# abdelhakim96/Dynamic-Obstacle-Avoidance-MPC

Measured on AMD Instinct MI355X. Metric: MPC solves/sec (N=20, 3 obstacles), higher is better.
Workload: dtype f64; 1 GPU; C2: 1024 identical scenarios per GPU, N=20, Tf=2s, 3 moving obstacles; global_batch=1024, per_gpu_batch=1024, N=20, n_obst=3, parallelism=single GPU

## Files before the change

### dynamic-obstacle-avoidance-mpc_amd/csrc/rti_kernel.hpp

```cpp
#pragma once
#include <hip/hip_runtime.h>
#include <stdint.h>
#include <type_traits>

#ifdef MPC_PHASE_TIMING
#define MPC_T0() long long t_prev_ = clock64()
#define MPC_TICK(k) do { const long long t_now_ = clock64(); tacc_[k] += t_now_ - t_prev_; t_prev_ = t_now_; } while (0)
#else
#define MPC_T0() do {} while (0)
#define MPC_TICK(k) do {} while (0)
#endif

namespace mpc {

struct World {
    double xmin, xmax, ymin, ymax;
    int bug_compat_predict;
};

enum : int {
    kFuseShift = 1,
    kFusePlant = 2,
    kFuseObstacles = 4,
    kFuseResetOnFail = 8,
    kFuseAliasBug = 16,
    kFuseMetrics = 32,
    kFuseInterpGuess = 64,
    kFuseAdvanceRef = 128
};

struct KParams {
    int N, batch;
    int n_obst;
    int soft_h, bx_terminal, iter_max;
    double dt, h2;
    double Hd_stage[7];
    double Hd_term[5];
    double Wg[6];
    double Weg[4];
    double bx_lo[4], bx_hi[4], bu_lo[2], bu_hi[2];
    double r2;
    double slack_a, slack_b, ss;
    double tol, mu0, thr0;
    double polish_ratio;
    float polish_tol;
    float polish_kappa;
    float polish_tol_unsolved;
    double polish_res_g;
    double tl_min;
    double mu_div, mu_cap, mu_settled;
    const double *x0, *P, *goal;
    const double *alpha;
    double *X, *U, *u0, *cost;
    int32_t *status, *iters;
    const int32_t *order;
    int32_t *iters_acc, *status_acc;
    const double *obst;
    double *x0_rw, *obst_rw;
    const double *noise;
    double randomness, vmax, tol_goal, r_hit;
    World world;
    int fused;
    double *ep_min_margin;
    int32_t *ep_flags;
    int32_t *ep_steps;
    double *trace;
    const double *yref;
    int32_t *ref_off;
    int ref_T;
};

__device__ __forceinline__ const double *ref_row(const double *yref, const int32_t *off, int T, int inst, int i)
{
    const int32_t *op = off;
    asm volatile("" : "+v"(op));
    const int o = off ? op[inst] : 0;
    int r = o > T - 1 - i ? T - 1 : o + i;
    r = r < 0 ? 0 : r;
    return yref + ((size_t)inst * T + r) * 6;
}

__device__ __forceinline__ void load_ref(const KParams &p, int inst, int i, bool has_u, double r[6])
{
    const double *row = ref_row(p.yref, p.ref_off, p.ref_T, inst, i);
#pragma unroll
    for (int c = 0; c < 4; c++) r[c] = row[c];
    r[4] = has_u ? row[4] : 0.0; r[5] = has_u ? row[5] : 0.0;
}

__device__ __forceinline__ double ls_cost_ref(const double Wg[6], const double Weg[4], const double xi[5], const double ui[2], const double r[6], bool has_u)
{
    const double ex = xi[0] - r[0], ey = xi[1] - r[1], ev = xi[3] - r[2], eo = xi[4] - r[3];
    if (has_u) {
        const double ea = ui[0] - r[4], eal = ui[1] - r[5];
        return 0.5 * (Wg[0] * ex * ex + Wg[1] * ey * ey + Wg[2] * ev * ev + Wg[3] * eo * eo + Wg[4] * ea * ea + Wg[5] * eal * eal);
    }
    return 0.5 * (Weg[0] * ex * ex + Weg[1] * ey * ey + Weg[2] * ev * ev + Weg[3] * eo * eo);
}

static constexpr double kTLMin = 1e-11;
static constexpr double kFracToBoundary = 0.999995;
static constexpr double kMuDiverged = 1e8;
static constexpr double kMuCapFailed = 1e4;
static constexpr int kMuCapSettled = 20;

__device__ static constexpr double kGLC[4] = {0.069431844202973712388, 0.330009478207571867599,
                                              0.669990521792428132401, 0.930568155797026287612};
__device__ static constexpr double kGLB[4] = {0.173927422568726928687, 0.326072577431273071313,
                                              0.326072577431273071313, 0.173927422568726928687};

template <bool JAC>
__device__ __forceinline__ void dyn_step(const double x[5], const double u[2], double dt, double xn[5], double ae[6], double be[4])
{
    const double psi = x[2], v = x[3], om = x[4], a = u[0], al = u[1];
    double sx = 0, sy = 0, xpsi = 0, xv = 0, xom = 0, xa = 0, xal = 0, ypsi = 0, yv = 0, yom = 0, ya = 0, yal = 0;
#pragma unroll
    for (int j = 0; j < 4; j++) {
        const double tau = kGLC[j] * dt, w = kGLB[j] * dt;
        const double vj = v + a * tau;
        const double pj = psi + om * tau + 0.5 * al * tau * tau;
        double sj, cj;
        sincos(pj, &sj, &cj);
        const double wvc = w * vj * cj, wvs = w * vj * sj;
        sx += wvc; sy += wvs;
        if (JAC) {
            const double ht2 = 0.5 * tau * tau;
            xpsi -= wvs;        ypsi += wvc;
            xv += w * cj;       yv += w * sj;
            xom -= wvs * tau;   yom += wvc * tau;
            xa += w * tau * cj; ya += w * tau * sj;
            xal -= wvs * ht2;   yal += wvc * ht2;
        }
    }
    xn[0] = x[0] + sx; xn[1] = x[1] + sy;
    xn[2] = psi + om * dt + 0.5 * al * dt * dt;
    xn[3] = v + a * dt;
    xn[4] = om + al * dt;
    if (JAC) {
        ae[0] = xpsi; ae[1] = xv; ae[2] = xom; ae[3] = ypsi; ae[4] = yv; ae[5] = yom;
        be[0] = xa; be[1] = xal; be[2] = ya; be[3] = yal;
    }
}

__device__ __forceinline__ void coord_advance(double lo, double hi, double dt, double &x, double &v)
{
#pragma clang fp contract(off)
    const double av = fabs(v);
    const double n = v < 0 ? x - lo : hi - x;
    bool hit = false;
    double t_hit = 0.0;
    if (v != 0 && !(n > av * dt * (1.0 + 0x1p-50))) { t_hit = n / av; hit = t_hit <= dt; }
    if (hit) { const double a = v * t_hit, b = v * (dt - t_hit); x = x + (a - b); v = -v; }
    else { const double a = v * dt; x = x + a; }
}
__device__ __forceinline__ void obstacle_advance(const World w, double dt, double &x, double &vx, double &y, double &vy)
{
    coord_advance(w.xmin, w.xmax, dt, x, vx);
    coord_advance(w.ymin, w.ymax, dt, y, vy);
}
__device__ __forceinline__ void interp_guess(const double x0[5], double goal_y, int i, int N, double xg[5])
{
#pragma clang fp contract(off)
    const double dy = goal_y - x0[1];
// ... 2865 lines not shown
```

### dynamic-obstacle-avoidance-mpc_amd/csrc/rti_split_kernel.hpp

```cpp
#pragma once
#include "rti_kernel.hpp"
#include <type_traits>

namespace mpc {

template <int LPS, int NOBST, bool W2 = false, bool BLK2 = false>
struct SplitLds {
    using LT = typename std::conditional<W2, RowLdsC, RowLds>::type;
    static constexpr int NBL = 6 / LPS;
    static constexpr int NSL = (NOBST + LPS - 1) / LPS;
    static __host__ __device__ constexpr int results(int N) { return W2 ? 0 : (N + 1) * RowLds::HS; }
    static __host__ __device__ constexpr int total(int N, bool lookahead)
    {
        if (BLK2) return Blk2Lds::total(N) + (lookahead ? (N + 1) * NOBST * 2 : 0);
        return LT::total(N, 1) + results(N) + ((lookahead && !W2) ? (N + 1) * NOBST * 2 : 0);
    }
};

template <int K>
__device__ __forceinline__ double nth_of_six(double a0, double a1, double a2, double a3, double a4, double a5)
{
    if constexpr (K == 0) return a0; else if constexpr (K == 1) return a1; else if constexpr (K == 2) return a2;
    else if constexpr (K == 3) return a3; else if constexpr (K == 4) return a4; else return a5;
}

#ifdef MPC_FORCE_WAVES2
#define MPC_SPLIT_BOUNDS(W2) __launch_bounds__(64, 2)
#else
#define MPC_SPLIT_BOUNDS(W2) __launch_bounds__(64, (W2) ? 2 : 1)
#endif
template <int NOBST, int LPS, bool W2 = false, bool MASKED = false, bool BLK2 = false, bool REF = false>
__global__ MPC_SPLIT_BOUNDS(W2) void rti_split_kernel(const KParams p)
{
    static_assert(!REF || !BLK2, "the per-stage reference is not built for the block-2 recursions");
    static_assert(LPS == 2 || LPS == 3, "two or three lanes per horizon stage");
    static_assert(!BLK2 || !W2, "the block-2 recursions exist on the dense layout only");
    using SL = SplitLds<LPS, NOBST, W2, BLK2>;
    using LT = typename SL::LT;
    constexpr int NBL = SL::NBL, NSL = SL::NSL;
    constexpr int kKK = 45;
    const int lane = threadIdx.x;
    const int inst = p.order ? p.order[blockIdx.x] : (int)blockIdx.x;
    const int N = p.N;
    const int nact = MASKED ? p.n_obst : NOBST;
    const int i = lane / LPS;
    const int h = lane - i * LPS;
    const bool own = (h == 0);
    const bool act = (i <= N);
    const bool has_u = (i < N);
    const bool xb = (i >= 1) && (i < N || (i == N && p.bx_terminal));
    const double dt = p.dt, h2 = p.h2;
    int is_part1 = (h == 1), is_part2 = (h == 2);
    asm volatile("" : "+v"(is_part1), "+v"(is_part2));
    auto part_of = [&](auto sc, double a0, double a1, double a2, double a3, double a4, double a5) {
        constexpr int s = decltype(sc)::value;
        double r = nth_of_six<s>(a0, a1, a2, a3, a4, a5);
        r = is_part1 ? nth_of_six<NBL + s>(a0, a1, a2, a3, a4, a5) : r;
        if (LPS == 3) r = is_part2 ? nth_of_six<(2 * NBL + s) % 6>(a0, a1, a2, a3, a4, a5) : r;
        return r;
    };
    auto zpart_of = [&](auto sc, double v0, double v1, double v2, double v3, double v5, double v6) {
        return part_of(sc, v0, v1, v2, v3, v5, v6);
    };
    using slot0 = std::integral_constant<int, 0>; using slot1 = std::integral_constant<int, 1>; using slot2 = std::integral_constant<int, 2>;
    auto slots_of = [&](const double (&v)[7], double (&out)[NBL]) {
        out[0] = zpart_of(slot0{}, v[0], v[1], v[2], v[3], v[5], v[6]);
        out[1] = zpart_of(slot1{}, v[0], v[1], v[2], v[3], v[5], v[6]);
        if constexpr (NBL > 2) out[2] = zpart_of(slot2{}, v[0], v[1], v[2], v[3], v[5], v[6]);
    };

#ifdef MPC_PHASE_TIMING
    long long tacc_[16] = {0, 0, 0, 0, 0, 0, 0, 0, 0, 0, 0, 0, 0, 0, 0, 0};
#endif
    MPC_T0();
    double x0v[5], gl[2];
#pragma unroll
    for (int c = 0; c < 5; c++) x0v[c] = p.x0[(size_t)inst * 5 + c];
    gl[0] = p.goal[(size_t)inst * 2]; gl[1] = p.goal[(size_t)inst * 2 + 1];
    if constexpr (W2) {
#pragma unroll
        for (int c = 0; c < 5; c++) x0v[c] = wave_uniform(x0v[c]);
        gl[0] = wave_uniform(gl[0]); gl[1] = wave_uniform(gl[1]);
    }
    double *Xg = p.X + (size_t)inst * (N + 1) * 5, *Ug = p.U + (size_t)inst * N * 2;
    const int ep_word = ((p.fused & kFuseMetrics) && p.ep_flags) ? p.ep_flags[inst] : 0;
    double xi[5] = {0, 0, 0, 0, 0}, ui[2] = {0, 0}, xnext[5] = {0, 0, 0, 0, 0};
    if (act) {
#pragma unroll
        for (int c = 0; c < 5; c++) xi[c] = Xg[i * 5 + c];
    }
    if (has_u) {
        ui[0] = Ug[i * 2]; ui[1] = Ug[i * 2 + 1];
#pragma unroll
        for (int c = 0; c < 5; c++) xnext[c] = Xg[(i + 1) * 5 + c];
    }
    extern __shared__ double lds_raw[];
    const LT RL = [&]() {
        if constexpr (W2) return RowLdsC(lds_raw + RowLdsC::CT + RowLdsC::pad_front(N), N, lds_raw);
        else return RowLds(lds_raw + RowLds::pad_front(N), N, lds_raw + RowLds::total(N, 1));
    }();
    const Blk2Lds BL(lds_raw, N);
    const RowLds RV(lds_raw, N / 2, BL.R);
    const int Mb = N >> 1;
    const int mblk = i >> 1;
    const bool odd = (i & 1) != 0;
    double *lds_P = BLK2 ? lds_raw + Blk2Lds::total(N) : (W2 ? RL.H : lds_raw + LT::total(N, 1) + SL::results(N));
    auto of_part = [&](double v, int q) { return q == 0 ? v : (q == 1 ? from_right(v) : from_right(from_right(v))); };
    double pxy[NSL][2];
    if (p.obst) {
        if (lane < 2 * nact) {
            const int j = lane >> 1, c = lane & 1;
            const double *o = p.obst + ((size_t)inst * nact + j) * 4;
            double q = o[c], v = (c == 0 && !p.world.bug_compat_predict) ? o[2] : o[3];
            const double lo = c ? p.world.ymin : p.world.xmin, hi = c ? p.world.ymax : p.world.xmax;
            lds_P[lane] = q;
            for (int k = 1; k <= N; k++) {
                coord_advance(lo, hi, dt, q, v);
                lds_P[k * NOBST * 2 + lane] = q;
            }
        }
        wave_sync();
    }
    MPC_TICK(10);
    if (p.obst) {
#pragma unroll
        for (int s = 0; s < NSL; s++) {
            const int j = s * LPS + h, jj = j < nact ? j : nact - 1;
            const double *src = lds_P + ((act ? i : 0) * NOBST + jj) * 2;
            pxy[s][0] = src[0]; pxy[s][1] = src[1];
        }
    } else {
#pragma unroll
        for (int s = 0; s < NSL; s++) {
            const int j = s * LPS + h, jj = j < nact ? j : nact - 1;
            const double *src = p.P + (((size_t)inst * (N + 1) + (act ? i : 0)) * nact + jj) * 2;
            pxy[s][0] = src[0]; pxy[s][1] = src[1];
        }
    }
    const bool ep_done = (ep_word & 1) != 0;
    double fin = gl[0] + gl[1] + ui[0] + ui[1];
#pragma unroll
    for (int c = 0; c < 5; c++) fin += x0v[c] + xi[c] + xnext[c];
#pragma unroll
    for (int s = 0; s < NSL; s++) fin += pxy[s][0] + pxy[s][1];

    MPC_TICK(11);
    double zpen = 0.0;
    {
        const double ex = x0v[0] - gl[0], ey = x0v[1] - gl[1];
        const double scale = p.slack_a * (ex * ex + ey * ey + x0v[3] * x0v[3] + x0v[4] * x0v[4] + p.slack_b);
        const double alpha_i = p.alpha ? p.alpha[(size_t)inst * (N + 1) + (act ? i : N)] : scale * (double)(N - i) / (double)N;
        zpen = alpha_i * (has_u ? p.ss : 1.0);
    }
    const bool vs = act && (i >= 1) && (p.soft_h ? (zpen > 0.0) : true);
    const bool soft = p.soft_h != 0;

    double lin0 = 0.0;
    double d0[5] = {0, 0, 0, 0, 0};
    StageLin S;
    S.a02 = S.a03 = S.a04 = S.a12 = S.a13 = S.a14 = S.b00 = S.b01 = S.b10 = S.b11 = 0.0; S.dt = dt; S.h2 = h2;
    double bb[5] = {0, 0, 0, 0, 0};
    if (has_u) {
        double xn[5], ae[6], be[4];
        dyn_step<true>(xi, ui, dt, xn, ae, be);
        S.a02 = ae[0]; S.a03 = ae[1]; S.a04 = ae[2]; S.a12 = ae[3]; S.a13 = ae[4]; S.a14 = ae[5];
        S.b00 = be[0]; S.b01 = be[1]; S.b10 = be[2]; S.b11 = be[3];
#pragma unroll
        for (int c = 0; c < 5; c++) { bb[c] = xn[c] - xnext[c]; lin0 = fmax(lin0, fabs(bb[c])); }
    }
    if (i == 0) {
#pragma unroll
        for (int c = 0; c < 5; c++) { d0[c] = x0v[c] - xi[c]; lin0 = fmax(lin0, fabs(d0[c])); }
    }
    StageLin Sa = S;
    double bba[5] = {0, 0, 0, 0, 0}, bh0[5] = {0, 0, 0, 0, 0};
    if constexpr (BLK2) {
        if (own && has_u) {
            double *w = BL.S + 16 * i;
            w[0] = bb[2]; w[1] = bb[3]; w[2] = S.a02; w[3] = S.a03; w[4] = S.a04; w[5] = bb[0]; w[6] = S.b00; w[7] = S.b01;
            w[8] = bb[4]; w[9] = 0.0; w[10] = S.a12; w[11] = S.a13; w[12] = S.a14; w[13] = bb[1]; w[14] = S.b10; w[15] = S.b11;
        }
        wave_sync();
        if (act && odd) {
            const double *w = BL.S + 16 * (i - 1);
            Sa.a02 = w[2]; Sa.a03 = w[3]; Sa.a04 = w[4]; Sa.b00 = w[6]; Sa.b01 = w[7];
            Sa.a12 = w[10]; Sa.a13 = w[11]; Sa.a14 = w[12]; Sa.b10 = w[14]; Sa.b11 = w[15];
            bba[0] = w[5]; bba[1] = w[13]; bba[2] = w[0]; bba[3] = w[1]; bba[4] = w[8];
        }
        if (own && odd && has_u) {
            const double Wh[5][10] = {
                {1.0, 0.0, Sa.a02 + S.a02, Sa.a03 + S.a03, fma(S.a02, dt, Sa.a04) + S.a04, 0.0,
                 fma(S.a03, dt, Sa.b00), fma(S.a04, dt, fma(S.a02, h2, Sa.b01)), S.b00, S.b01},
                {0.0, 1.0, Sa.a12 + S.a12, Sa.a13 + S.a13, fma(S.a12, dt, Sa.a14) + S.a14, 0.0,
                 fma(S.a13, dt, Sa.b10), fma(S.a14, dt, fma(S.a12, h2, Sa.b11)), S.b10, S.b11},
                {0.0, 0.0, 1.0, 0.0, 2.0 * dt, 0.0, 0.0, fma(dt, dt, h2), 0.0, h2},
                {0.0, 0.0, 0.0, 1.0, 0.0, 0.0, dt, 0.0, dt, 0.0},
                {0.0, 0.0, 0.0, 0.0, 1.0, 0.0, 0.0, dt, 0.0, dt}};
            double *w = BL.W + Blk2Lds::WS * mblk;
#pragma unroll
            for (int k = 0; k < 5; k++)
#pragma unroll
                for (int c = 0; c < 10; c++) w[k * 10 + c] = Wh[k][c];
            bh0[0] = fma(S.a04, bba[4], fma(S.a03, bba[3], fma(S.a02, bba[2], bba[0]))) + bb[0];
            bh0[1] = fma(S.a14, bba[4], fma(S.a13, bba[3], fma(S.a12, bba[2], bba[1]))) + bb[1];
            bh0[2] = fma(dt, bba[4], bba[2]) + bb[2]; bh0[3] = bba[3] + bb[3]; bh0[4] = bba[4] + bb[4];
        }
        if (own && act && (odd || i == N)) {
            double *hc = BL.H + Blk2Lds::HS * mblk;
#pragma unroll
            for (int e = 0; e < 100; e++) hc[e] = 0.0;
        }
    } else
    if constexpr (W2) {
        if (own && act) { double *hc = RL.H + LT::HS * i; hc[49] = 0.0; hc[50] = 0.0; }
        if (lane < 8) {
            const double c2[8] = {0.0, 0.0, 1.0, 0.0, dt, 0.0, 0.0, h2}, c3[8] = {0.0, 0.0, 0.0, 1.0, 0.0, 0.0, dt, 0.0}, c4[8] = {0.0, 0.0, 0.0, 0.0, 1.0, 0.0, 0.0, dt};
            double v2 = 0.0, v3 = 0.0, v4 = 0.0;
#pragma unroll
            for (int c = 0; c < 8; c++) if (lane == c) { v2 = c2[c]; v3 = c3[c]; v4 = c4[c]; }
            RL.C[3 * lane] = v2; RL.C[3 * lane + 1] = v3; RL.C[3 * lane + 2] = v4;
        }
        if (own && has_u) {
            double *w = RL.W + LT::WS * i;
            const double Wrow[2][8] = {{1.0, 0.0, S.a02, S.a03, S.a04, 0.0, S.b00, S.b01}, {0.0, 1.0, S.a12, S.a13, S.a14, 0.0, S.b10, S.b11}};
#pragma unroll
            for (int k = 0; k < 2; k++)
#pragma unroll
                for (int c = 0; c < 8; c++) w[k * 8 + c] = Wrow[k][c];
        }
    } else {
    if (own && act) {
        double *hc = RL.H + LT::HS * i;
#pragma unroll
        for (int e = 0; e < 64; e++) hc[e] = 0.0;
    }
    if (own && has_u) {
        double *w = RL.W + LT::WS * i;
        const double Wrow[5][8] = {{1.0, 0.0, S.a02, S.a03, S.a04, 0.0, S.b00, S.b01}, {0.0, 1.0, S.a12, S.a13, S.a14, 0.0, S.b10, S.b11},
                                   {0.0, 0.0, 1.0, 0.0, dt, 0.0, 0.0, h2}, {0.0, 0.0, 0.0, 1.0, 0.0, 0.0, dt, 0.0}, {0.0, 0.0, 0.0, 0.0, 1.0, 0.0, 0.0, dt}};
#pragma unroll
        for (int k = 0; k < 5; k++)
#pragma unroll
            for (int c = 0; c < 8; c++) w[k * 8 + c] = Wrow[k][c];
    }
    }

    MPC_TICK(12);
    bool bp[NBL];
    double cl0[NBL], ch0[NBL], hq[NBL], hd[NBL], gc0[NBL];
    double ll[NBL], tl[NBL], lh[NBL], th[NBL], rtl[NBL], rth[NBL], zs[NBL];
    double yr[REF ? 6 : 1];
    if constexpr (REF) load_ref(p, inst, act ? i : N, has_u, yr);
    {
        auto slot_init = [&](auto sc) {
            constexpr int s = decltype(sc)::value;
            const double val = part_of(sc, ui[0], ui[1], xi[0], xi[1], xi[3], xi[4]);
            const double lo = part_of(sc, p.bu_lo[0], p.bu_lo[1], p.bx_lo[0], p.bx_lo[1], p.bx_lo[2], p.bx_lo[3]);
            const double hi = part_of(sc, p.bu_hi[0], p.bu_hi[1], p.bx_hi[0], p.bx_hi[1], p.bx_hi[2], p.bx_hi[3]);
            const bool is_u = part_of(sc, 1.0, 1.0, 0.0, 0.0, 0.0, 0.0) != 0.0;
            bp[s] = act && (is_u ? has_u : xb);
            hd[s] = part_of(sc, has_u ? p.Hd_stage[0] : 0.0, has_u ? p.Hd_stage[1] : 0.0, has_u ? p.Hd_stage[2] : p.Hd_term[0],
                            has_u ? p.Hd_stage[3] : p.Hd_term[1], has_u ? p.Hd_stage[5] : p.Hd_term[3], has_u ? p.Hd_stage[6] : p.Hd_term[4]);
            hq[s] = (is_u && !has_u) ? 1.0 : hd[s];
            const double wg = part_of(sc, has_u ? p.Wg[4] : 0.0, has_u ? p.Wg[5] : 0.0, has_u ? p.Wg[0] : p.Weg[0], has_u ? p.Wg[1] : p.Weg[1],
                                      has_u ? p.Wg[2] : p.Weg[2], has_u ? p.Wg[3] : p.Weg[3]);
            if constexpr (REF) gc0[s] = wg * (val - part_of(sc, yr[4], yr[5], yr[0], yr[1], yr[2], yr[3]));
            else gc0[s] = wg * (val - part_of(sc, 0.0, 0.0, gl[0], gl[1], 0.0, 0.0));
            cl0[s] = val - lo; ch0[s] = hi - val;
            tl[s] = fmax(cl0[s], p.thr0); th[s] = fmax(ch0[s], p.thr0);
            rtl[s] = rcp_nr(tl[s]); rth[s] = rcp_nr(th[s]);
            ll[s] = p.mu0 * rtl[s]; lh[s] = p.mu0 * rth[s];
            zs[s] = 0.0;
            if (bp[s]) lin0 = fmax(lin0, fmax(tl[s] - cl0[s], th[s] - ch0[s]));
        };
        slot_init(std::integral_constant<int, 0>{});
        slot_init(std::integral_constant<int, 1>{});
        if constexpr (NBL > 2) slot_init(std::integral_constant<int, 2>{});
    }
    const double hd_psi = has_u ? p.Hd_stage[4] : p.Hd_term[2];
    bool sp[NSL];
    double hh[NSL], ax[NSL], ay[NSL], sv[NSL], l1[NSL], t1[NSL], l2[NSL], t2[NSL], rt1[NSL], rt2[NSL];
#pragma unroll
    for (int s = 0; s < NSL; s++) {
        sp[s] = vs && (s * LPS + h < nact);
        const double ex = xi[0] - pxy[s][0], ey = xi[1] - pxy[s][1];
        hh[s] = ex * ex + ey * ey - p.r2; ax[s] = 2 * ex; ay[s] = 2 * ey;
        if (soft) {
            sv[s] = (hh[s] < 0 ? -hh[s] : 0.0) + p.thr0;
            t1[s] = fmax(hh[s] + sv[s], p.thr0);
            t2[s] = fmax(sv[s], p.thr0);
        } else {
            sv[s] = 0.0; t1[s] = fmax(hh[s], p.thr0); t2[s] = 1.0;
            if (sp[s]) lin0 = fmax(lin0, t1[s] - hh[s]);
        }
        rt1[s] = rcp_nr(t1[s]); rt2[s] = rcp_nr(t2[s]);
        l1[s] = p.mu0 * rt1[s]; l2[s] = soft ? p.mu0 * rt2[s] : 0.0;
    }
    int n_items_lane = 0;
#pragma unroll
    for (int s = 0; s < NBL; s++) n_items_lane += bp[s] ? 2 : 0;
#pragma unroll
    for (int s = 0; s < NSL; s++) n_items_lane += sp[s] ? (soft ? 2 : 1) : 0;
    const double n_items = seg_sum<64>((double)n_items_lane, lane);
    const double inv_items = wave_uniform(n_items > 0 ? 1.0 / n_items : 0.0);
    if (!(fabs(fin) <= 1e300)) lin0 = INFINITY;
    lin0 = wave_uniform(seg_max<64>(lin0, lane));

    double z[7] = {0, 0, 0, 0, 0, 0, 0};
    double rhoPi = 1.0;
    int it = 0;
    IpmState ipm;
    ipm.running = !ep_done;
    int &status = ipm.status, &it_done = ipm.it_done;
    bool &running = ipm.running;
    float stepl = 0.0f;
    if (!(lin0 <= 1e300)) { status = 4; running = false; }

    auto stationarity = [&]() {
        double gsh[NBL], gk[6] = {0, 0, 0, 0, 0, 0}, sx = 0.0, sy = 0.0, rsm = 0.0;
#pragma unroll
        for (int s = 0; s < NBL; s++) { gsh[s] = gc0[s] + hd[s] * zs[s] + (bp[s] ? lh[s] - ll[s] : 0.0); gk[s] = gsh[s]; }
#pragma unroll
        for (int s = 0; s < NSL; s++) if (sp[s]) {
            sx -= l1[s] * ax[s]; sy -= l1[s] * ay[s];
            if (soft) rsm = fmax(rsm, fabs(zpen * sv[s] + zpen - l1[s] - l2[s]));
        }
        double shx = sx, shy = sy;
#pragma unroll
        for (int q = 1; q < LPS; q++) {
#pragma unroll
            for (int s = 0; s < NBL; s++) gsh[s] = from_right(gsh[s]);
            shx = from_right(shx); shy = from_right(shy);
#pragma unroll
            for (int s = 0; s < NBL; s++) gk[q * NBL + s] = gsh[s];
            sx += shx; sy += shy;
        }
        const double g[7] = {gk[0], gk[1], gk[2] + sx, gk[3] + sy, hd_psi * z[4], gk[4], gk[5]};
        const double ru = adjoint_inputs<64>(own && act, own && has_u, S, g, lane);
        return wave_uniform(seg_max<64>(fmax(ru, rsm), lane));
    };
    MPC_TICK(13);
    for (it = 0;; it++) {
        double msum = 0.0, cmax = 0.0;
#pragma unroll
        for (int s = 0; s < NBL; s++) if (bp[s]) {
            const double a = ll[s] * tl[s], b = lh[s] * th[s];
            msum += a + b;
            if (!(tl[s] <= 2 * p.tl_min || ll[s] <= 2 * p.tl_min)) cmax = fmax(cmax, a);
            if (!(th[s] <= 2 * p.tl_min || lh[s] <= 2 * p.tl_min)) cmax = fmax(cmax, b);
        }
#pragma unroll
        for (int s = 0; s < NSL; s++) if (sp[s]) {
            const double a = l1[s] * t1[s];
            msum += a;
            if (!(t1[s] <= 2 * p.tl_min || l1[s] <= 2 * p.tl_min)) cmax = fmax(cmax, a);
            if (soft) {
                const double b = l2[s] * t2[s];
                msum += b;
                if (!(t2[s] <= 2 * p.tl_min || l2[s] <= 2 * p.tl_min)) cmax = fmax(cmax, b);
            }
        }
        seg_reduce2<64, true>(msum, cmax, lane);
        const double mu = msum * inv_items;
        const double lin = rhoPi * lin0;
        ipm_head(p, ipm, it, mu, lin, cmax);
        if (__ballot(ipm.ask_g) != 0ull) ipm_head_g(p, ipm, it, stationarity());
        if (!running) break;
        ipm.cprev = wave_uniform(cmax);
        MPC_TICK(0);

        double rdl[NBL], rdh[NBL];
        struct SoftT { double w1, w2, rD, be1, be2, rs, rd1, rd2; } so[NSL];
        double hdiag_[NBL], g_[NBL], ssum[5];
        {
#pragma unroll
            for (int s = 0; s < NBL; s++) {
                rdl[s] = (cl0[s] + zs[s]) - tl[s];
                rdh[s] = (ch0[s] - zs[s]) - th[s];
                double hdiag = hq[s], g = gc0[s] + hd[s] * zs[s];
                if (bp[s]) {
                    const double wl = ll[s] * rtl[s], wh = lh[s] * rth[s];
                    const double bl = (ll[s] * tl[s] + ll[s] * rdl[s]) * rtl[s], bh = (lh[s] * th[s] + lh[s] * rdh[s]) * rth[s];
                    hdiag += wl + wh;
                    g += lh[s] - ll[s];
                    g += bl - bh;
                }
                hdiag_[s] = hdiag; g_[s] = g;
            }
            double sxx = 0.0, syy = 0.0, sxy = 0.0, glx = 0.0, gly = 0.0, cbx = 0.0, cby = 0.0;
#pragma unroll
            for (int s = 0; s < NSL; s++) {
                SoftT &o = so[s];
                const double y = ax[s] * z[2] + ay[s] * z[3];
                o.w1 = l1[s] * rt1[s];
                if (soft) {
                    o.rd1 = (hh[s] + y + sv[s]) - t1[s]; o.rd2 = sv[s] - t2[s];
                    o.be1 = (l1[s] * t1[s] + l1[s] * o.rd1) * rt1[s];
                    o.w2 = l2[s] * rt2[s];
                    o.be2 = (l2[s] * t2[s] + l2[s] * o.rd2) * rt2[s];
                    o.rs = zpen * sv[s] + zpen - l1[s] - l2[s];
                    o.rD = rcp_nr(zpen + o.w1 + o.w2);
                } else {
                    o.rd1 = (hh[s] + y) - t1[s]; o.rd2 = 0.0;
                    o.be1 = (l1[s] * t1[s] + l1[s] * o.rd1) * rt1[s];
                    o.w2 = 0.0; o.be2 = 0.0; o.rs = 0.0; o.rD = 0.0;
// ... 399 lines not shown
                rowpar_vector_fast<false>(lane, Mb, RV, lane < 16);
                wave_sync();
                if (own && odd && has_u) {
                    const double *pp = BL.R + Blk2Lds::RS * (mblk + 1) + RowVec::P;
                    const double pv[5] = {pp[0], pp[1], pp[2], pp[3], pp[4]};
                    const double wv[5] = {pv[0], pv[1], S.dpsi(pv), S.dv(pv), S.dom(pv)};
                    const double ma0 = gu[0] + Sa.dua(wv), ma1 = gu[1] + Sa.dual(wv), mb0 = gu[2] + S.dua(pv), mb1 = gu[3] + S.dual(pv);
                    const double y0 = mb0, y1 = fma(-fac[4], y0, mb1), y2 = fma(-fac[7], y1, fma(-fac[5], y0, ma0)), y3 = fma(-fac[9], y2, fma(-fac[8], y1, fma(-fac[6], y0, ma1)));
                    const double k3 = -(y3 * fac[3]);
                    const double k2 = fma(-fac[9], k3, -(y2 * fac[2]));
                    const double k1 = fma(-fac[8], k3, fma(-fac[7], k2, -(y1 * fac[1])));
                    const double k0 = fma(-fac[6], k3, fma(-fac[5], k2, fma(-fac[4], k1, -(y0 * fac[0]))));
                    const double kc[4] = {k2, k3, k0, k1};
                    const double B0[4] = {fma(S.a03, dt, Sa.b00), fma(S.a04, dt, fma(S.a02, h2, Sa.b01)), S.b00, S.b01};
                    const double B1[4] = {fma(S.a13, dt, Sa.b10), fma(S.a14, dt, fma(S.a12, h2, Sa.b11)), S.b10, S.b11};
                    double *cc = BL.R + Blk2Lds::RS * mblk + RowVec::ACL + 5;
                    cc[0 * RowVec::RS] = fma(B0[3], kc[3], fma(B0[2], kc[2], fma(B0[1], kc[1], B0[0] * kc[0])));
                    cc[1 * RowVec::RS] = fma(B1[3], kc[3], fma(B1[2], kc[2], fma(B1[1], kc[1], B1[0] * kc[0])));
                    cc[2 * RowVec::RS] = fma(h2, kc[3], fma(dt, dt, h2) * kc[1]);
                    cc[3 * RowVec::RS] = fma(dt, kc[2], dt * kc[0]);
                    cc[4 * RowVec::RS] = fma(dt, kc[3], dt * kc[1]);
                    double *kk = BL.R + Blk2Lds::RS * mblk + kKK;
                    kk[0] = kc[0]; kk[1] = kc[1]; kk[2] = kc[2]; kk[4] = kc[3];
                }
            } else {
            if (own && act) {
                double *cc = RL.R + LT::HS * i + RowVec::CT;
#pragma unroll
                for (int c = 0; c < 5; c++) cc[c] = gc[2 + c] + F.K0[c] * gc[0] + F.K1[c] * gc[1];
            }
            wave_sync();
            rowpar_vector_fast<false>(lane, N, RL, lane < 16);
            wave_sync();
            if (has_u) {
                const double *pp = RL.R + LT::HS * (i + 1) + RowVec::P;
                const double pv[5] = {pp[0], pp[1], pp[2], pp[3], pp[4]};
                const double m0 = gc[0] + S.dua(pv), m1 = gc[1] + S.dual(pv);
                F.k1 = fma(F.l, m0, -m1) * F.i11;
                F.k0 = fma(-F.l, F.k1, -(m0 * F.i00));
            }
            }
        }
        MPC_TICK(6);
        double dz[7] = {0, 0, 0, 0, 0, 0, 0};
        if constexpr (BLK2) {
            if (lane == 0) {
#pragma unroll
                for (int c = 0; c < 5; c++) BL.R[RowVec::X + c] = 0.0;
            }
            wave_sync();
            rowpar_vector_fast<true>(lane, Mb, RV, lane < 16);
            wave_sync();
            if (has_u) {
                const double *kk = BL.R + Blk2Lds::RS * mblk + kKK;
                kh[0] = kk[0]; kh[1] = kk[1]; kh[2] = kk[2]; kh[3] = kk[4];
            }
            const double zero5[5] = {0, 0, 0, 0, 0};
            pair_step(zero5, dz);
        } else {
        if (own && has_u) {
            double *cc = RL.R + LT::HS * i + RowVec::ACL + 5;
            cc[0 * RowVec::RS] = S.b00 * F.k0 + S.b01 * F.k1; cc[1 * RowVec::RS] = S.b10 * F.k0 + S.b11 * F.k1;
            cc[2 * RowVec::RS] = h2 * F.k1; cc[3 * RowVec::RS] = dt * F.k0; cc[4 * RowVec::RS] = dt * F.k1;
            RL.R[LT::HS * i + kKK] = F.k0; RL.R[LT::HS * i + kKK + 1] = F.k1;
        }
        if (lane == 0) {
#pragma unroll
            for (int c = 0; c < 5; c++) RL.R[RowVec::X + c] = 0.0;
        }
        wave_sync();
        rowpar_vector_fast<true>(lane, N, RL, lane < 16);
        wave_sync();
        if (act) {
            const double *xx = RL.R + LT::HS * i + RowVec::X;
            double u0 = has_u ? RL.R[LT::HS * i + kKK] : 0.0, u1 = has_u ? RL.R[LT::HS * i + kKK + 1] : 0.0;
#pragma unroll
            for (int c = 0; c < 5; c++) { dz[2 + c] = xx[c]; u0 += F.K0[c] * xx[c]; u1 += F.K1[c] * xx[c]; }
            dz[0] = u0; dz[1] = u1;
        }
        }
#pragma unroll
        for (int c = 0; c < 7; c++) dz[c] += za[c];
        MPC_TICK(7);

        {
            double rmax = 0.0, rmaxd = 0.0;
            double dzs[NBL], dtl_[NBL], dth_[NBL], dll_[NBL], dlh_[NBL];
            slots_of(dz, dzs);
#pragma unroll
            for (int s = 0; s < NBL; s++) {
                dtl_[s] = dzs[s] + rdl[s]; dth_[s] = -dzs[s] + rdh[s];
                dll_[s] = -(ll[s] * tl[s] - smu + ppl[s] + ll[s] * dtl_[s]) * rtl[s];
                dlh_[s] = -(lh[s] * th[s] - smu + pph[s] + lh[s] * dth_[s]) * rth[s];
                if (bp[s]) {
                    rmax = fmax(rmax, fmax(-dtl_[s] * rtl[s], -dth_[s] * rth[s]));
                    rmaxd = fmax(rmaxd, fmax(-dll_[s] * rcp_nr(ll[s]), -dlh_[s] * rcp_nr(lh[s])));
                }
            }
            double dt1_[NSL], dl1_[NSL], dt2_[NSL], dl2_[NSL], ds_[NSL];
#pragma unroll
            for (int s = 0; s < NSL; s++) {
                const SoftT &o = so[s];
                const double y = ax[s] * dz[2] + ay[s] * dz[3];
                dt2_[s] = dl2_[s] = ds_[s] = 0.0;
                if (soft) {
                    const double db1 = (pp1[s] - smu) * rt1[s], db2 = (pp2[s] - smu) * rt2[s];
                    const double rsum = o.rs + (o.be1 + db1) + (o.be2 + db2);
                    ds_[s] = -(rsum + o.w1 * y) * o.rD;
                    dt1_[s] = o.rd1 + (y * (zpen + o.w2) - rsum) * o.rD;
                    dt2_[s] = o.rd2 + ds_[s];
                    dl2_[s] = -(l2[s] * t2[s] - smu + pp2[s] + l2[s] * dt2_[s]) * rt2[s];
                    if (sp[s]) { rmax = fmax(rmax, -dt2_[s] * rt2[s]); rmaxd = fmax(rmaxd, -dl2_[s] * rcp_nr(l2[s])); }
                } else dt1_[s] = o.rd1 + y;
                dl1_[s] = -(l1[s] * t1[s] - smu + pp1[s] + l1[s] * dt1_[s]) * rt1[s];
                if (sp[s]) { rmax = fmax(rmax, -dt1_[s] * rt1[s]); rmaxd = fmax(rmaxd, -dl1_[s] * rcp_nr(l1[s])); }
            }
            seg_reduce2<64, false>(rmax, rmaxd, lane);
            double alpha, alphad;
            ipm_step_lengths(rmax, rmaxd, alpha, alphad);
#ifndef MPC_PHASE_TIMING
            if (p.trace && lane == 0) p.trace[((size_t)inst * p.iter_max + it) * 4 + 2] = alpha;
#endif
            ipm_step_check(ipm, it, alpha, alphad, smu);
            ipm_polish_step<64>(p, ipm, lane, alpha, dz, stepl);
            if (running) {
#pragma unroll
                for (int c = 0; c < 7; c++) z[c] += alpha * dz[c];
#pragma unroll
                for (int s = 0; s < NBL; s++) {
                    zs[s] += alpha * dzs[s];
                    if (bp[s]) {
                        tl[s] = fmax(tl[s] + alpha * dtl_[s], p.tl_min); th[s] = fmax(th[s] + alpha * dth_[s], p.tl_min);
                        ll[s] = fmax(ll[s] + alphad * dll_[s], p.tl_min); lh[s] = fmax(lh[s] + alphad * dlh_[s], p.tl_min);
                        rtl[s] = rcp_nr(tl[s]); rth[s] = rcp_nr(th[s]);
                    }
                }
#pragma unroll
                for (int s = 0; s < NSL; s++) if (sp[s]) {
                    t1[s] = fmax(t1[s] + alpha * dt1_[s], p.tl_min); l1[s] = fmax(l1[s] + alphad * dl1_[s], p.tl_min);
                    rt1[s] = rcp_nr(t1[s]);
                    if (soft) {
                        sv[s] += alpha * ds_[s];
                        t2[s] = fmax(t2[s] + alpha * dt2_[s], p.tl_min); l2[s] = fmax(l2[s] + alphad * dl2_[s], p.tl_min);
                        rt2[s] = rcp_nr(t2[s]);
                    }
                }
                rhoPi = wave_uniform(rhoPi * (1.0 - alpha));
            }
        }
        MPC_TICK(8);
        if (!running) break;
    }

    if constexpr (!W2) {
        const double *xg = p.x0 + (size_t)inst * 5, *gg = p.goal + (size_t)inst * 2;
        asm volatile("" : "+v"(xg), "+v"(gg));
#pragma unroll
        for (int c = 0; c < 5; c++) x0v[c] = xg[c];
        gl[0] = gg[0]; gl[1] = gg[1];
    }
    const bool store = !ep_done;
    status = ipm_finite_step<64>(status, z, lane);
    if (status != 4) {
#pragma unroll
        for (int c = 0; c < 5; c++) xi[c] += z[2 + c];
        ui[0] += z[0]; ui[1] += z[1];
    }
    const double u_apply[2] = {lane_value(ui[0], 0), lane_value(ui[1], 0)};
    if ((p.fused & kFuseResetOnFail) && status == 4) {
        xi[0] = x0v[0]; xi[1] = x0v[1]; xi[2] = x0v[2]; xi[3] = 0.0; xi[4] = 0.0; ui[0] = ui[1] = 0.0;
        if (p.fused & kFuseInterpGuess) interp_guess(x0v, gl[1], i <= N ? i : N, N, xi);
    }
    if (store && own && (status != 4 || (p.fused & (kFuseResetOnFail | kFuseShift)))) {
        if (p.fused & kFuseShift) {
            if (act && i >= 1) {
#pragma unroll
                for (int c = 0; c < 5; c++) Xg[(i - 1) * 5 + c] = xi[c];
            }
            if (i == N) {
#pragma unroll
                for (int c = 0; c < 5; c++) Xg[N * 5 + c] = xi[c];
            }
            if (has_u && i >= 1) { Ug[(i - 1) * 2] = ui[0]; Ug[(i - 1) * 2 + 1] = ui[1]; }
            if (i == 0) { Ug[(N - 1) * 2] = 0.0; Ug[(N - 1) * 2 + 1] = 0.0; }
        } else {
            if (act) {
#pragma unroll
                for (int c = 0; c < 5; c++) Xg[i * 5 + c] = xi[c];
            }
            if (has_u) { Ug[i * 2] = ui[0]; Ug[i * 2 + 1] = ui[1]; }
        }
    }
    if (p.fused & (kFusePlant | kFuseObstacles | kFuseMetrics)) {
        double xp[5] = {x0v[0], x0v[1], x0v[2], x0v[3], x0v[4]};
        if ((p.fused & kFuseAliasBug) && (p.fused & kFuseResetOnFail) && status == 4) { xp[3] = 0.0; xp[4] = 0.0; }
        double xnew[5] = {xp[0], xp[1], xp[2], xp[3], xp[4]};
        if (p.fused & kFusePlant) dyn_step<false>(xp, u_apply, dt, xnew, nullptr, nullptr);
        if ((p.fused & kFusePlant) && lane == 0 && store && p.x0_rw) {
#pragma unroll
            for (int c = 0; c < 5; c++) p.x0_rw[(size_t)inst * 5 + c] = xnew[c];
        }
        double margin = INFINITY;
        if (p.obst && lane < nact) {
            const double *o = p.obst + ((size_t)inst * nact + lane) * 4;
            double ox = o[0], oy = o[1], ovx = o[2], ovy = o[3];
            if (p.fused & kFuseObstacles) {
                if (p.noise) obstacle_noise(p.randomness, p.vmax, p.noise[((size_t)inst * nact + lane) * 2], p.noise[((size_t)inst * nact + lane) * 2 + 1], ovx, ovy);
                obstacle_advance(p.world, dt, ox, ovx, oy, ovy);
                if (store && p.obst_rw) { double *w = p.obst_rw + ((size_t)inst * nact + lane) * 4; w[0] = ox; w[1] = oy; w[2] = ovx; w[3] = ovy; }
            }
            const double ddx = xnew[0] - ox, ddy = xnew[1] - oy;
            margin = sqrt(ddx * ddx + ddy * ddy) - p.r_hit;
        }
        if (p.fused & kFuseMetrics) {
            margin = -seg_max<64>(-margin, lane);
            if (lane == 0 && store) {
                int fl = p.ep_flags[inst];
                if (xnew[0] < p.world.xmin || xnew[0] > p.world.xmax || xnew[1] < p.world.ymin || xnew[1] > p.world.ymax) fl |= 2;
                const double mm = fmin(p.ep_min_margin[inst], margin);
                p.ep_min_margin[inst] = mm;
                if (mm <= 0.0) fl |= 4;
                const double gx_ = xnew[0] - gl[0], gy_ = xnew[1] - gl[1];
                if (sqrt(gx_ * gx_ + gy_ * gy_) <= p.tol_goal) fl |= 1;
                else p.ep_steps[inst] += 1;
                p.ep_flags[inst] = fl;
            }
        }
    }
    if (lane == 0 && p.u0 && store) { p.u0[(size_t)inst * 2] = u_apply[0]; p.u0[(size_t)inst * 2 + 1] = u_apply[1]; }
    if (p.cost) {
        double J = 0.0;
        if (act) {
            if (REF && own) {
                const double *row = ref_row(p.yref, p.ref_off, p.ref_T, inst, i);
                const double r[6] = {row[0], row[1], row[2], row[3], has_u ? row[4] : 0.0, has_u ? row[5] : 0.0};
                J = ls_cost_ref(p.Wg, p.Weg, xi, ui, r, has_u);
            } else if (own) {
                const double ex = xi[0] - gl[0], ey = xi[1] - gl[1];
                if (has_u) J = 0.5 * (p.Wg[0] * ex * ex + p.Wg[1] * ey * ey + p.Wg[2] * xi[3] * xi[3] + p.Wg[3] * xi[4] * xi[4]
                                      + p.Wg[4] * ui[0] * ui[0] + p.Wg[5] * ui[1] * ui[1]);
                else J = 0.5 * (p.Weg[0] * ex * ex + p.Weg[1] * ey * ey + p.Weg[2] * xi[3] * xi[3] + p.Weg[3] * xi[4] * xi[4]);
            }
#pragma unroll
            for (int s = 0; s < NSL; s++) if (s * LPS + h < nact) {
                const double dx = xi[0] - pxy[s][0], dy = xi[1] - pxy[s][1];
                const double hv = dx * dx + dy * dy - p.r2;
                const double v = hv < 0 ? -hv : 0.0;
                J += zpen * (v + 0.5 * v * v);
            }
        }
        J = seg_sum<64>(J, lane);
        if (lane == 0 && store) p.cost[inst] = J;
    }
    if (lane == 0 && store) {
        if (p.iters_acc) p.iters_acc[inst] += it_done;
        if (p.status_acc) p.status_acc[inst] += (status == 4 ? 1 : 0) + (status == 2 ? 65536 : 0);
        if (p.status) p.status[inst] = status;
        if (p.iters) p.iters[inst] = it_done;
    }
    if constexpr (REF) {
        if ((p.fused & kFuseAdvanceRef) && lane == 0 && store && p.ref_off) p.ref_off[inst] += 1;
    }
#ifdef MPC_PHASE_TIMING
    __builtin_amdgcn_s_waitcnt(0);
    MPC_TICK(14);
    if (p.trace && lane == 0) { for (int k = 0; k < 16; k++) p.trace[((size_t)inst * p.iter_max) * 4 + k] = (double)tacc_[k]; }
#endif
}

}
```

Measured before the change: 7.164 million solves/s.

## Prefetch epilogue state into LDS at kernel start and fuse final reductions

For the non-W2 split kernel, the obstacle states, noise, episode metrics, accumulators and reference offset are loaded from global memory at kernel entry. They are stashed in an LDS area appended to the shared layout, so the epilogue reads them from LDS instead of issuing dependent global loads after the solve. The epilogue is restructured: read-modify-write accumulators become plain stores computed from the prefetched values, and the cost sum and margin max are merged into one two-value segmented reduction. This removes global load latency from the tail, at the cost of extra LDS, more live registers early in the kernel, and a duplicated epilogue path. Extra timing ticks are added for profiling builds.

```diff
diff --git a/dynamic-obstacle-avoidance-mpc_amd/csrc/rti_kernel.hpp b/dynamic-obstacle-avoidance-mpc_amd/csrc/rti_kernel.hpp
--- a/dynamic-obstacle-avoidance-mpc_amd/csrc/rti_kernel.hpp
+++ b/dynamic-obstacle-avoidance-mpc_amd/csrc/rti_kernel.hpp
@@ -6,9 +6,11 @@
 #ifdef MPC_PHASE_TIMING
 #define MPC_T0() long long t_prev_ = clock64()
 #define MPC_TICK(k) do { const long long t_now_ = clock64(); tacc_[k] += t_now_ - t_prev_; t_prev_ = t_now_; } while (0)
+#define MPC_TICK_DRAINED(k) do { __builtin_amdgcn_s_waitcnt(0); MPC_TICK(k); } while (0)
 #else
 #define MPC_T0() do {} while (0)
 #define MPC_TICK(k) do {} while (0)
+#define MPC_TICK_DRAINED(k) do {} while (0)
 #endif
 
 namespace mpc {
diff --git a/dynamic-obstacle-avoidance-mpc_amd/csrc/rti_split_kernel.hpp b/dynamic-obstacle-avoidance-mpc_amd/csrc/rti_split_kernel.hpp
--- a/dynamic-obstacle-avoidance-mpc_amd/csrc/rti_split_kernel.hpp
+++ b/dynamic-obstacle-avoidance-mpc_amd/csrc/rti_split_kernel.hpp
@@ -10,10 +10,12 @@
     static constexpr int NBL = 6 / LPS;
     static constexpr int NSL = (NOBST + LPS - 1) / LPS;
     static __host__ __device__ constexpr int results(int N) { return W2 ? 0 : (N + 1) * RowLds::HS; }
+    static constexpr int ST_X0 = 0, ST_GOAL = 5, ST_MARGIN = 7, ST_INTS = 8, ST_OBST = 12, ST_NOISE = 12 + 4 * NOBST;
+    static constexpr int STASH = W2 ? 0 : 12 + 6 * NOBST;
     static __host__ __device__ constexpr int total(int N, bool lookahead)
     {
-        if (BLK2) return Blk2Lds::total(N) + (lookahead ? (N + 1) * NOBST * 2 : 0);
-        return LT::total(N, 1) + results(N) + ((lookahead && !W2) ? (N + 1) * NOBST * 2 : 0);
+        if (BLK2) return Blk2Lds::total(N) + (lookahead ? (N + 1) * NOBST * 2 : 0) + STASH;
+        return LT::total(N, 1) + results(N) + ((lookahead && !W2) ? (N + 1) * NOBST * 2 : 0) + STASH;
     }
 };
 
@@ -35,6 +37,7 @@
     static_assert(!REF || !BLK2, "the per-stage reference is not built for the block-2 recursions");
     static_assert(LPS == 2 || LPS == 3, "two or three lanes per horizon stage");
     static_assert(!BLK2 || !W2, "the block-2 recursions exist on the dense layout only");
+    static_assert(4 * NOBST <= 64, "one lane per word of the obstacle states");
     using SL = SplitLds<LPS, NOBST, W2, BLK2>;
     using LT = typename SL::LT;
     constexpr int NBL = SL::NBL, NSL = SL::NSL;
@@ -70,9 +73,18 @@
     };
 
 #ifdef MPC_PHASE_TIMING
-    long long tacc_[16] = {0, 0, 0, 0, 0, 0, 0, 0, 0, 0, 0, 0, 0, 0, 0, 0};
+    long long tacc_[32];
+#pragma unroll
+    for (int k = 0; k < 32; k++) tacc_[k] = 0;
 #endif
     MPC_T0();
+    const bool fuse_noise = !W2 && p.obst && p.noise && (p.fused & kFuseObstacles);
+    const bool fuse_metrics = (p.fused & kFuseMetrics) && p.ep_flags;
+    double st_obst = 0.0, st_noise = 0.0, st_margin = 0.0;
+    int st_steps = 0, st_iacc = 0, st_sacc = 0, st_roff = 0;
+    if constexpr (!W2) {
+        if (p.obst && lane < 4 * nact) st_obst = p.obst[(size_t)inst * nact * 4 + lane];
+    }
     double x0v[5], gl[2];
 #pragma unroll
     for (int c = 0; c < 5; c++) x0v[c] = p.x0[(size_t)inst * 5 + c];
@@ -83,7 +95,21 @@
         gl[0] = wave_uniform(gl[0]); gl[1] = wave_uniform(gl[1]);
     }
     double *Xg = p.X + (size_t)inst * (N + 1) * 5, *Ug = p.U + (size_t)inst * N * 2;
-    const int ep_word = ((p.fused & kFuseMetrics) && p.ep_flags) ? p.ep_flags[inst] : 0;
+    auto ep_flags_opaque = [&]() { const int32_t *v = p.ep_flags; asm volatile("" : "+v"(v)); return v[inst]; };
+    const int ep_word = ((p.fused & kFuseMetrics) && p.ep_flags) ? (W2 ? p.ep_flags[inst] : ep_flags_opaque()) : 0;
+    if constexpr (!W2) {
+        if (fuse_noise && lane < 2 * nact) st_noise = p.noise[(size_t)inst * nact * 2 + lane];
+        if (lane == 0) {
+            if (fuse_metrics) { st_margin = p.ep_min_margin[inst]; st_steps = p.ep_steps[inst]; }
+            if (p.iters_acc) st_iacc = p.iters_acc[inst];
+            if (p.status_acc) st_sacc = p.status_acc[inst];
+        }
+        if constexpr (REF) {
+            const int32_t *op = p.ref_off;
+            asm volatile("" : "+v"(op));
+            if (p.ref_off) st_roff = op[inst];
+        }
+    }
     double xi[5] = {0, 0, 0, 0, 0}, ui[2] = {0, 0}, xnext[5] = {0, 0, 0, 0, 0};
     if (act) {
 #pragma unroll
@@ -94,7 +120,10 @@
 #pragma unroll
         for (int c = 0; c < 5; c++) xnext[c] = Xg[(i + 1) * 5 + c];
     }
+    MPC_TICK_DRAINED(16);
     extern __shared__ double lds_raw[];
+    double *lds_S = W2 ? lds_raw : lds_raw + SL::total(N, p.obst != nullptr) - SL::STASH;
+    int32_t *lds_SI = reinterpret_cast<int32_t *>(lds_S + SL::ST_INTS);
     const LT RL = [&]() {
         if constexpr (W2) return RowLdsC(lds_raw + RowLdsC::CT + RowLdsC::pad_front(N), N, lds_raw);
         else return RowLds(lds_raw + RowLds::pad_front(N), N, lds_raw + RowLds::total(N, 1));
@@ -108,18 +137,36 @@
     auto of_part = [&](double v, int q) { return q == 0 ? v : (q == 1 ? from_right(v) : from_right(from_right(v))); };
     double pxy[NSL][2];
     if (p.obst) {
+        if constexpr (!W2) {
+            if (lane < 4 * nact) lds_S[SL::ST_OBST + lane] = st_obst;
+            wave_sync();
+        }
         if (lane < 2 * nact) {
             const int j = lane >> 1, c = lane & 1;
-            const double *o = p.obst + ((size_t)inst * nact + j) * 4;
+            const double *o = W2 ? p.obst + ((size_t)inst * nact + j) * 4 : lds_S + SL::ST_OBST + j * 4;
             double q = o[c], v = (c == 0 && !p.world.bug_compat_predict) ? o[2] : o[3];
             const double lo = c ? p.world.ymin : p.world.xmin, hi = c ? p.world.ymax : p.world.xmax;
+            MPC_TICK_DRAINED(17);
             lds_P[lane] = q;
             for (int k = 1; k <= N; k++) {
                 coord_advance(lo, hi, dt, q, v);
                 lds_P[k * NOBST * 2 + lane] = q;
             }
+            MPC_TICK(18);
         }
         wave_sync();
+    }
+    int ep_word_u = ep_word;
+    if constexpr (!W2) {
+        ep_word_u = __builtin_amdgcn_readfirstlane(ep_word);
+        if (fuse_noise && lane < 2 * nact) lds_S[SL::ST_NOISE + lane] = st_noise;
+        if (lane == 0) {
+#pragma unroll
+            for (int c = 0; c < 5; c++) lds_S[SL::ST_X0 + c] = x0v[c];
+            lds_S[SL::ST_GOAL] = gl[0]; lds_S[SL::ST_GOAL + 1] = gl[1];
+            lds_S[SL::ST_MARGIN] = st_margin;
+            lds_SI[0] = ep_word_u; lds_SI[1] = st_steps; lds_SI[2] = st_iacc; lds_SI[3] = st_sacc; lds_SI[4] = st_roff;
+        }
     }
     MPC_TICK(10);
     if (p.obst) {
@@ -137,7 +184,7 @@
             pxy[s][0] = src[0]; pxy[s][1] = src[1];
         }
     }
-    const bool ep_done = (ep_word & 1) != 0;
+    const bool ep_done = ((W2 ? ep_word : ep_word_u) & 1) != 0;
     double fin = gl[0] + gl[1] + ui[0] + ui[1];
 #pragma unroll
     for (int c = 0; c < 5; c++) fin += x0v[c] + xi[c] + xnext[c];
@@ -174,6 +221,7 @@
     }
     StageLin Sa = S;
     double bba[5] = {0, 0, 0, 0, 0}, bh0[5] = {0, 0, 0, 0, 0};
+    MPC_TICK(19);
     if constexpr (BLK2) {
         if (own && has_u) {
             double *w = BL.S + 16 * i;
@@ -250,7 +298,18 @@
     double cl0[NBL], ch0[NBL], hq[NBL], hd[NBL], gc0[NBL];
     double ll[NBL], tl[NBL], lh[NBL], th[NBL], rtl[NBL], rth[NBL], zs[NBL];
     double yr[REF ? 6 : 1];
-    if constexpr (REF) load_ref(p, inst, act ? i : N, has_u, yr);
+    auto ref_row_at = [&](int off, int k) {
+        int r = off > p.ref_T - 1 - k ? p.ref_T - 1 : off + k;
+        r = r < 0 ? 0 : r;
+        return p.yref + ((size_t)inst * p.ref_T + r) * 6;
+    };
+    if constexpr (REF && W2) load_ref(p, inst, act ? i : N, has_u, yr);
+    else if constexpr (REF) {
+        const double *row = ref_row_at(st_roff, act ? i : N);
+#pragma unroll
+        for (int c = 0; c < 4; c++) yr[c] = row[c];
+        yr[4] = has_u ? row[4] : 0.0; yr[5] = has_u ? row[5] : 0.0;
+    }
     {
         auto slot_init = [&](auto sc) {
             constexpr int s = decltype(sc)::value;
@@ -956,13 +1015,8 @@
         if (!running) break;
     }
 
-    if constexpr (!W2) {
-        const double *xg = p.x0 + (size_t)inst * 5, *gg = p.goal + (size_t)inst * 2;
-        asm volatile("" : "+v"(xg), "+v"(gg));
-#pragma unroll
-        for (int c = 0; c < 5; c++) x0v[c] = xg[c];
-        gl[0] = gg[0]; gl[1] = gg[1];
-    }
+    if constexpr (W2) {
+    MPC_TICK_DRAINED(20);
     const bool store = !ep_done;
     status = ipm_finite_step<64>(status, z, lane);
     if (status != 4) {
@@ -995,6 +1049,7 @@
             if (has_u) { Ug[i * 2] = ui[0]; Ug[i * 2 + 1] = ui[1]; }
         }
     }
+    MPC_TICK(21);
     if (p.fused & (kFusePlant | kFuseObstacles | kFuseMetrics)) {
         double xp[5] = {x0v[0], x0v[1], x0v[2], x0v[3], x0v[4]};
         if ((p.fused & kFuseAliasBug) && (p.fused & kFuseResetOnFail) && status == 4) { xp[3] = 0.0; xp[4] = 0.0; }
@@ -1004,6 +1059,7 @@
 #pragma unroll
             for (int c = 0; c < 5; c++) p.x0_rw[(size_t)inst * 5 + c] = xnew[c];
         }
+        MPC_TICK(22);
         double margin = INFINITY;
         if (p.obst && lane < nact) {
             const double *o = p.obst + ((size_t)inst * nact + lane) * 4;
@@ -1016,6 +1072,7 @@
             const double ddx = xnew[0] - ox, ddy = xnew[1] - oy;
             margin = sqrt(ddx * ddx + ddy * ddy) - p.r_hit;
         }
+        MPC_TICK(23);
         if (p.fused & kFuseMetrics) {
             margin = -seg_max<64>(-margin, lane);
             if (lane == 0 && store) {
@@ -1030,6 +1087,7 @@
                 p.ep_flags[inst] = fl;
             }
         }
+        MPC_TICK(24);
     }
     if (lane == 0 && p.u0 && store) { p.u0[(size_t)inst * 2] = u_apply[0]; p.u0[(size_t)inst * 2 + 1] = u_apply[1]; }
     if (p.cost) {
@@ -1056,6 +1114,7 @@
         J = seg_sum<64>(J, lane);
         if (lane == 0 && store) p.cost[inst] = J;
     }
+    MPC_TICK(25);
     if (lane == 0 && store) {
         if (p.iters_acc) p.iters_acc[inst] += it_done;
         if (p.status_acc) p.status_acc[inst] += (status == 4 ? 1 : 0) + (status == 2 ? 65536 : 0);
@@ -1065,10 +1124,142 @@
     if constexpr (REF) {
         if ((p.fused & kFuseAdvanceRef) && lane == 0 && store && p.ref_off) p.ref_off[inst] += 1;
     }
+    } else {
+    const bool store = !ep_done;
+    const bool fuse_step = (p.fused & (kFusePlant | kFuseObstacles | kFuseMetrics)) != 0;
+    const bool obst_lane = fuse_step && p.obst && lane < nact;
+#pragma unroll
+    for (int c = 0; c < 5; c++) x0v[c] = lds_S[SL::ST_X0 + c];
+    gl[0] = lds_S[SL::ST_GOAL]; gl[1] = lds_S[SL::ST_GOAL + 1];
+    double ox = 0.0, oy = 0.0, ovx = 0.0, ovy = 0.0, nzx = 0.0, nzy = 0.0;
+    if (obst_lane) {
+        const double *o = lds_S + SL::ST_OBST + lane * 4;
+        ox = o[0]; oy = o[1]; ovx = o[2]; ovy = o[3];
+        if (fuse_noise) { nzx = lds_S[SL::ST_NOISE + lane * 2]; nzy = lds_S[SL::ST_NOISE + lane * 2 + 1]; }
+    }
+    const double ep_margin0 = lds_S[SL::ST_MARGIN];
+    const int ep_flags0 = lds_SI[0], ep_steps0 = lds_SI[1], iacc0 = lds_SI[2], sacc0 = lds_SI[3];
+    double yc[REF ? 6 : 1];
+    if constexpr (REF) {
+        if (p.cost && act && own) {
+            const double *row = ref_row_at(lds_SI[4], i);
+#pragma unroll
+            for (int c = 0; c < 6; c++) yc[c] = row[c];
+        }
+    }
+    MPC_TICK_DRAINED(20);
+    status = ipm_finite_step<64>(status, z, lane);
+    if (status != 4) {
+#pragma unroll
+        for (int c = 0; c < 5; c++) xi[c] += z[2 + c];
+        ui[0] += z[0]; ui[1] += z[1];
+    }
+    const double u_apply[2] = {lane_value(ui[0], 0), lane_value(ui[1], 0)};
+    if ((p.fused & kFuseResetOnFail) && status == 4) {
+        xi[0] = x0v[0]; xi[1] = x0v[1]; xi[2] = x0v[2]; xi[3] = 0.0; xi[4] = 0.0; ui[0] = ui[1] = 0.0;
+        if (p.fused & kFuseInterpGuess) interp_guess(x0v, gl[1], i <= N ? i : N, N, xi);
+    }
+    if (store && own && (status != 4 || (p.fused & (kFuseResetOnFail | kFuseShift)))) {
+        if (p.fused & kFuseShift) {
+            if (act && i >= 1) {
+#pragma unroll
+                for (int c = 0; c < 5; c++) Xg[(i - 1) * 5 + c] = xi[c];
+            }
+            if (i == N) {
+#pragma unroll
+                for (int c = 0; c < 5; c++) Xg[N * 5 + c] = xi[c];
+            }
+            if (has_u && i >= 1) { Ug[(i - 1) * 2] = ui[0]; Ug[(i - 1) * 2 + 1] = ui[1]; }
+            if (i == 0) { Ug[(N - 1) * 2] = 0.0; Ug[(N - 1) * 2 + 1] = 0.0; }
+        } else {
+            if (act) {
+#pragma unroll
+                for (int c = 0; c < 5; c++) Xg[i * 5 + c] = xi[c];
+            }
+            if (has_u) { Ug[i * 2] = ui[0]; Ug[i * 2 + 1] = ui[1]; }
+        }
+    }
+    if (lane == 0 && store) {
+        if (p.u0) { p.u0[(size_t)inst * 2] = u_apply[0]; p.u0[(size_t)inst * 2 + 1] = u_apply[1]; }
+        if (p.iters_acc) p.iters_acc[inst] = iacc0 + it_done;
+        if (p.status_acc) p.status_acc[inst] = sacc0 + (status == 4 ? 1 : 0) + (status == 2 ? 65536 : 0);
+        if (p.status) p.status[inst] = status;
+        if (p.iters) p.iters[inst] = it_done;
+        if constexpr (REF) {
+            if ((p.fused & kFuseAdvanceRef) && p.ref_off) p.ref_off[inst] = lds_SI[4] + 1;
+        }
+    }
+    MPC_TICK(21);
+    double xnew[5] = {x0v[0], x0v[1], x0v[2], x0v[3], x0v[4]};
+    double margin = INFINITY;
+    if (fuse_step) {
+        double xp[5] = {x0v[0], x0v[1], x0v[2], x0v[3], x0v[4]};
+        if ((p.fused & kFuseAliasBug) && (p.fused & kFuseResetOnFail) && status == 4) { xp[3] = 0.0; xp[4] = 0.0; }
+#pragma unroll
+        for (int c = 0; c < 5; c++) xnew[c] = xp[c];
+        if (p.fused & kFusePlant) dyn_step<false>(xp, u_apply, dt, xnew, nullptr, nullptr);
+        if ((p.fused & kFusePlant) && lane == 0 && store && p.x0_rw) {
+#pragma unroll
+            for (int c = 0; c < 5; c++) p.x0_rw[(size_t)inst * 5 + c] = xnew[c];
+        }
+        MPC_TICK(22);
+        if (obst_lane) {
+            if (p.fused & kFuseObstacles) {
+                if (fuse_noise) obstacle_noise(p.randomness, p.vmax, nzx, nzy, ovx, ovy);
+                obstacle_advance(p.world, dt, ox, ovx, oy, ovy);
+                if (store && p.obst_rw) { double *w = p.obst_rw + ((size_t)inst * nact + lane) * 4; w[0] = ox; w[1] = oy; w[2] = ovx; w[3] = ovy; }
+            }
+            const double ddx = xnew[0] - ox, ddy = xnew[1] - oy;
+            margin = sqrt(ddx * ddx + ddy * ddy) - p.r_hit;
+        }
+        MPC_TICK(23);
+    }
+    double J = 0.0;
+    if (p.cost && act) {
+        if (REF && own) {
+            const double r[6] = {yc[0], yc[1], yc[2], yc[3], has_u ? yc[4] : 0.0, has_u ? yc[5] : 0.0};
+            J = ls_cost_ref(p.Wg, p.Weg, xi, ui, r, has_u);
+        } else if (own) {
+            const double ex = xi[0] - gl[0], ey = xi[1] - gl[1];
+            if (has_u) J = 0.5 * (p.Wg[0] * ex * ex + p.Wg[1] * ey * ey + p.Wg[2] * xi[3] * xi[3] + p.Wg[3] * xi[4] * xi[4]
+                                  + p.Wg[4] * ui[0] * ui[0] + p.Wg[5] * ui[1] * ui[1]);
+            else J = 0.5 * (p.Weg[0] * ex * ex + p.Weg[1] * ey * ey + p.Weg[2] * xi[3] * xi[3] + p.Weg[3] * xi[4] * xi[4]);
+        }
+#pragma unroll
+        for (int s = 0; s < NSL; s++) if (s * LPS + h < nact) {
+            const double dx = xi[0] - pxy[s][0], dy = xi[1] - pxy[s][1];
+            const double hv = dx * dx + dy * dy - p.r2;
+            const double v = hv < 0 ? -hv : 0.0;
+            J += zpen * (v + 0.5 * v * v);
+        }
+    }
+    MPC_TICK(25);
+    const bool metrics = fuse_step && (p.fused & kFuseMetrics);
+    double negm = -margin;
+    if (p.cost && metrics) seg_reduce2<64, true>(J, negm, lane);
+    else if (p.cost) J = seg_sum<64>(J, lane);
+    else if (metrics) negm = seg_max<64>(negm, lane);
+    margin = -negm;
+    if (lane == 0 && store) {
+        if (p.cost) p.cost[inst] = J;
+        if (metrics) {
+            int fl = ep_flags0;
+            if (xnew[0] < p.world.xmin || xnew[0] > p.world.xmax || xnew[1] < p.world.ymin || xnew[1] > p.world.ymax) fl |= 2;
+            const double mm = fmin(ep_margin0, margin);
+            p.ep_min_margin[inst] = mm;
+            if (mm <= 0.0) fl |= 4;
+            const double gx_ = xnew[0] - gl[0], gy_ = xnew[1] - gl[1];
+            if (sqrt(gx_ * gx_ + gy_ * gy_) <= p.tol_goal) fl |= 1;
+            else p.ep_steps[inst] = ep_steps0 + 1;
+            p.ep_flags[inst] = fl;
+        }
+    }
+    MPC_TICK(24);
+    }
 #ifdef MPC_PHASE_TIMING
     __builtin_amdgcn_s_waitcnt(0);
     MPC_TICK(14);
-    if (p.trace && lane == 0) { for (int k = 0; k < 16; k++) p.trace[((size_t)inst * p.iter_max) * 4 + k] = (double)tacc_[k]; }
+    if (p.trace && lane == 0) { for (int k = 0; k < 32 && k < 4 * p.iter_max; k++) p.trace[((size_t)inst * p.iter_max) * 4 + k] = (double)tacc_[k]; }
 #endif
 }
 
```

New measurement: 7.193 million solves/s, median of 6. About the same (+0.4%).
